# cherubicXN/neat

Measured on AMD Instinct MI355X. Metric: ray-samples/s (train step) on ABC-neat-a, higher is better.
Workload: dtype bf16; 1 GPU; C2: abc-neat-a networks, 1024 rays x 128 samples per GPU, depth samples given, train step = forward + loss + backward + Adam; rays_per_gpu=1024, samples_per_ray=128, global_rays=1024, parallelism=dp1, weights=synthetic 'rough' (seed 42), launch=hip graph replay, the whole step one launch (forward + loss + backward + Adam)

## Files before the change

### neat_amd/csrc/bf16_common.hpp

```cpp
#pragma once
#include <hip/hip_runtime.h>
#include <stdint.h>

#ifndef NEAT_HALF
#define NEAT_HALF 0
#endif

namespace neat {

struct DevOnce {
  unsigned long long mask = 0;
  static int dev() { int d = 0; if (hipGetDevice(&d) != hipSuccess || d < 0 || d > 63) d = 0; return d; }
  operator bool() const { return ((mask >> dev()) & 1ull) != 0; }
  DevOnce& operator=(bool v) { if (v) mask |= 1ull << dev(); else mask &= ~(1ull << dev()); return *this; }
};
#define NEAT_TRY(expr) do { hipError_t e_ = (expr); if (e_ != hipSuccess) return e_; } while (0)
template <auto... Kerns> hipError_t lds_limit(int bytes) {
  static DevOnce done;
  if (done) return hipSuccess;
  hipError_t e = hipSuccess;
  ((e = e != hipSuccess ? e : hipFuncSetAttribute(reinterpret_cast<const void*>(Kerns), hipFuncAttributeMaxDynamicSharedMemorySize, bytes)), ...);
  if (e == hipSuccess) done = true;
  return e;
}
// ... 80 lines not shown

struct FusedArgs {
  const float* x_fm; int P, ldp;
  const uint4* Wp[9]; int KS[9]; const float* bias[9];
  int save, values_only;
  u16* h[9];
  float* E;
  u16* feat; float* sdfraw;
  const uint4* Wlo[9]; u16* hlo[9]; u16* featlo;
  float* sdf_out;
  float radius, scale;
  int bias8_rot, bias8_n;
  const int* gate; int gate_value;
};

struct AdjArgs {
  int P, ldp;
  const uint4* Wp[8];
  const u16* h[9];
  u16* u[8];
  const float* w8; const float* rs8;
  float* es; float* e0;
  const uint4* Wlo[8]; const u16* hlo[9];
};

struct HeadX3Args {
  int P, ldp;
  int nvalid;
  const u16* feat; const u16* featlo;
  const float* small; int srows;
  const uint4* Wp[5]; const uint4* Wlo[5];
  const float* bias[5];
  u16* hid[5];
  float* out;
  const u16* smallbf;
  u16* mask[5];
};

// ... 15 lines not shown
```

### neat_amd/csrc/kernels.hpp

```cpp
#pragma once
#include <hip/hip_runtime.h>
#include <stdint.h>
#include "bf16_common.hpp"
#include "device_util.hpp"

namespace neat {

constexpr int BM = 64;
constexpr int WG = 256;

__device__ __forceinline__ float softplus100(float a) {
  const float t = 100.0f * a;
  return t > 20.0f ? a : log1pf(expf(t)) * 0.01f;
}
__device__ __forceinline__ float dphi_from_h(float h) { return -expm1f(-100.0f * h); }

enum Epi : int {
  EPI_LINEAR = 0,
  EPI_SOFTPLUS = 1,
  EPI_RELU = 2,
  EPI_SIGMOID = 3,
  EPI_REV = 4,
  EPI_TAN = 5,
  EPI_BWD = 6,
// ... 596 lines not shown
      f *= 2.0f;
    }
  }
}

__global__ void adjoint_seed_kernel(const float* __restrict__ v8, const float* __restrict__ rs8,
                                    const float* __restrict__ h8, int ldp, float* __restrict__ u7) {
  const int p = blockIdx.x * blockDim.x + threadIdx.x;
  const int n = blockIdx.y;
  if (p >= ldp) return;
  const float w = v8[n] * rs8[0];
  const size_t idx = (size_t)n * ldp + p;
  u7[idx] = w * dphi_from_h(h8[idx]);
}

struct HeadInArgs { const float* dirs; int P, S; float* small_r; float* small_a; u16* bf_r; u16* bf_a;
                    int skip_fp32 = 0; };
template <bool FAST>
__global__ void sdf_finalize_kernel(const float* __restrict__ x_fm, const float* __restrict__ out8,
                                    const float* __restrict__ e0, const float* __restrict__ es, int P, int ldp,
                                    float radius, float scale, float* __restrict__ sdf, float* __restrict__ g_fm,
                                    float* __restrict__ mask, float* __restrict__ sdf_rm, float* __restrict__ g_rm,
                                    int n_clamp, float* __restrict__ g_extra_rm, const float* __restrict__ E, HeadInArgs hin) {
  const int p = blockIdx.x * blockDim.x + threadIdx.x;
  if (p >= ldp) return;
  float xv[3], gv[3] = {0.f, 0.f, 0.f};
#pragma unroll
  for (int c = 0; c < 3; ++c) xv[c] = x_fm[(size_t)c * ldp + p];
  float s = out8[p], m = 0.0f;
  if (e0) {
#pragma unroll
    for (int c = 0; c < 3; ++c) {
      float acc = e0[(size_t)c * ldp + p] + es[(size_t)c * ldp + p];
      float f = 1.0f;
#pragma unroll
      for (int k = 0; k < 6; ++k) {
        const float es_ = e0[(size_t)(3 + 6 * k + c) * ldp + p] + es[(size_t)(3 + 6 * k + c) * ldp + p];
        const float ec_ = e0[(size_t)(6 + 6 * k + c) * ldp + p] + es[(size_t)(6 + 6 * k + c) * ldp + p];
        const float ang = xv[c] * f;
        if (E) acc += f * E[(size_t)(6 + 6 * k + c) * ldp + p] * es_ - f * E[(size_t)(3 + 6 * k + c) * ldp + p] * ec_;
        else acc += f * (FAST ? __cosf(ang) : cosf(ang)) * es_ - f * (FAST ? __sinf(ang) : sinf(ang)) * ec_;
        f *= 2.0f;
      }
      gv[c] = acc;
    }
  }
  if (radius > 0.0f && p < n_clamp) {
    const float nr = sqrtf(xv[0] * xv[0] + xv[1] * xv[1] + xv[2] * xv[2]);
    const float sph = scale * (radius - nr);
    if (sph < s) {
      s = sph; m = 1.0f;
      const float inv = nr > 0.0f ? -scale / nr : 0.0f;
      gv[0] = xv[0] * inv; gv[1] = xv[1] * inv; gv[2] = xv[2] * inv;
    }
  }
  sdf[p] = s;
  if (mask) mask[p] = m;
  if (g_fm) { g_fm[p] = gv[0]; g_fm[(size_t)ldp + p] = gv[1]; g_fm[(size_t)2 * ldp + p] = gv[2]; }
  if (hin.small_r) {
    const int r = (p < hin.P ? p : 0) / hin.S;
    float vr[40], va[16];
#pragma unroll
    for (int i = 0; i < 40; ++i) vr[i] = 0.0f;
#pragma unroll
    for (int i = 0; i < 16; ++i) va[i] = 0.0f;
#pragma unroll
    for (int c = 0; c < 3; ++c) {
      const float xc = xv[c], gc = gv[c];
      const float dc = (p < hin.P) ? hin.dirs[r * 3 + c] : 0.0f;
      vr[c] = xc; vr[3 + c] = dc;
      float f = 1.0f;
#pragma unroll
      for (int k = 0; k < 4; ++k) {
        vr[6 + 6 * k + c] = sinf(dc * f);
        vr[9 + 6 * k + c] = cosf(dc * f);
        f *= 2.0f;
      }
      vr[30 + c] = gc;
      va[c] = xc; va[3 + c] = dc; va[6 + c] = gc;
    }
    if (!hin.skip_fp32) {
#pragma unroll
      for (int i = 0; i < 33; ++i) hin.small_r[(size_t)i * ldp + p] = vr[i];
#pragma unroll
      for (int i = 0; i < 9; ++i) hin.small_a[(size_t)i * ldp + p] = va[i];
    }
    if (hin.bf_r) {
#pragma unroll
      for (int o = 0; o < 5; ++o)
        reinterpret_cast<uint4*>(hin.bf_r)[(size_t)o * ldp + p] = make_uint4(pack2(vr[8 * o], vr[8 * o + 1]), pack2(vr[8 * o + 2], vr[8 * o + 3]),
                                                                            pack2(vr[8 * o + 4], vr[8 * o + 5]), pack2(vr[8 * o + 6], vr[8 * o + 7]));
    }
    if (hin.bf_a) {
#pragma unroll
// ... 319 lines not shown
```

### neat_amd/csrc/kernels_fused.hpp

```cpp
#pragma once
#include "bf16_common.hpp"
#include "fused_launch.hpp"
#include <type_traits>

namespace neat {

#ifndef NEAT_F6_ABLATE
#define NEAT_F6_ABLATE 0
#endif
#ifndef NEAT_ADJ_ABLATE
#define NEAT_ADJ_ABLATE 0
#endif
#ifndef NEAT_ADJ_NT_LOAD
#define NEAT_ADJ_NT_LOAD 1
#endif
#ifndef NEAT_F6_WIDE
#define NEAT_F6_WIDE 1
#endif
#ifndef NEAT_ADJ_WIDE
#define NEAT_ADJ_WIDE 1
#endif
#ifndef NEAT_F6_SPLITK
#define NEAT_F6_SPLITK 0
#endif
// ... 45 lines not shown
}
__device__ __forceinline__ void f6_store16(void* p, uint4 v) {
  typedef unsigned v4u_t __attribute__((ext_vector_type(4)));
  const v4u_t w = {v.x, v.y, v.z, v.w};
  if (NEAT_F6_NT) __builtin_nontemporal_store(w, reinterpret_cast<v4u_t*>(p));
  else *reinterpret_cast<v4u_t*>(p) = w;
}
__device__ __forceinline__ void f6_store8(void* p, uint2 v) {
  typedef unsigned long long u64_t;
  if (NEAT_F6_NT) __builtin_nontemporal_store(__builtin_bit_cast(u64_t, v), reinterpret_cast<u64_t*>(p));
  else *reinterpret_cast<uint2*>(p) = v;
}

template <bool ACT_, bool SAVE_, int N_, int DST_, int BIASOFF_, bool UDOM_ = false> struct F6EpiCfg {
  static constexpr bool ACT = ACT_, SAVE = SAVE_, NONE = false, REV = false, UDOM = UDOM_;
  static constexpr int N = N_, DST = DST_, BIASOFF = BIASOFF_, SPLIT = 1 << 30;
};
struct F6NoEpi { static constexpr bool ACT = false, SAVE = false, NONE = true, REV = false, UDOM = false; static constexpr int N = 256, DST = 0, BIASOFF = 0, SPLIT = 1 << 30; };
template <bool SAVE_, int N_, int DST_, int SPLIT_> struct F6RevCfg {
  static constexpr bool ACT = false, SAVE = SAVE_, NONE = false, REV = true, UDOM = false;
  static constexpr int N = N_, DST = DST_, BIASOFF = 0, SPLIT = SPLIT_;
};

template <class E, int RT> __device__ __forceinline__ void f6_load_bias(const F6Lane& L, float4 (&bq)[4 * RT]) {
#pragma unroll
  for (int g = 0; g < 4 * RT; ++g) bq[g] = *reinterpret_cast<const float4*>(L.bias + (E::BIASOFF + (g >> 2) * 32 + 8 * (g & 3)) * 4);
}

template <class E, int RT> __device__ __forceinline__ void f6_load_bias16(const F6Lane& L, f32x16 (&c0)[RT]) {
#pragma unroll
  for (int g = 0; g < 4 * RT; ++g) {
    const float4 b = *reinterpret_cast<const float4*>(L.bias + (E::BIASOFF + (g >> 2) * 32 + 8 * (g & 3)) * 4);
    c0[g >> 2][4 * (g & 3) + 0] = b.x; c0[g >> 2][4 * (g & 3) + 1] = b.y; c0[g >> 2][4 * (g & 3) + 2] = b.z; c0[g >> 2][4 * (g & 3) + 3] = b.w;
  }
}

// ... 20 lines not shown
          }
          hw = st.hs[2 * (q & 1) + pr];
        } else hw = __float_as_uint(pr ? bq[g].y : bq[g].x);
        st.m0 = x0 * dphi_fast(bf_lo(hw));
        st.m1 = x1 * dphi_fast(bf_hi(hw));
      }
      return;
    }
    float r0 = st.m0, r1 = st.m1;
    if (E::SPLIT < 256 && 32 * (RT * wave + i) + 8 * q + 7 >= E::SPLIT) {
      int hio = hi;
      asm volatile("" : "+v"(hio));
      const int n0 = 32 * (RT * wave + i) + 8 * q + 4 * hio + 2 * pr;
      const bool st_ok = FULL || t < nt;
      const unsigned col = L.fcol + t * 32, ld = L.ldp16 >> 4;
      if (n0 >= E::SPLIT) { r0 = 0.0f; if (st_ok && n0 < E::N) f6_storef(L.frows + (unsigned)(n0 - E::SPLIT) * ld + col, x0); }
      if (n0 + 1 >= E::SPLIT) { r1 = 0.0f; if (st_ok && n0 + 1 < E::N) f6_storef(L.frows + (unsigned)(n0 + 1 - E::SPLIT) * ld + col, x1); }
    }
    const unsigned pk = pack2(r0, r1);
    if (pr == 0) { st.lo = pk; return; }
    const uint2 v = make_uint2(st.lo, pk);
    if (E::SPLIT > 0) *reinterpret_cast<uint2*>(L.quad[E::DST] + ((i * 4 + q) * BP + t * 32) * 16) = v;
    if (E::SAVE && (FULL || t < nt) && !(NEAT_ADJ_ABLATE & 1)) {
      if (NEAT_ADJ_WIDE) {
        if (q & 1) f6_store16(reinterpret_cast<char*>(hout) + ((unsigned)(i * 4 + q - 1) * L.ldp16 + L.goct) + t * 512, f6_octet(st.vprev, v));
        else st.vprev = v;
      } else f6_store8(reinterpret_cast<char*>(hout) + ((unsigned)(i * 4 + q) * L.ldp16 + L.gquad) + t * 512, v);
    }
    return;
  }
  if (h == 0) {
    if (E::ACT && NEAT_F6_ABLATE != 1) {
// ... 374 lines not shown
          sv = fminf(sv, a.scale * (a.radius - sqrtf(x0 * x0 + x1 * x1 + x2 * x2)));
        }
        if (p < a.P) a.sdf_out[p] = sv;
      } else {
        a.sdfraw[p] = sv;
      }
    }
    __syncthreads();
   }
  }
}

#ifndef NEAT_ADJ_SINGLE
#define NEAT_ADJ_SINGLE 1
#endif
template <bool SAVE>
__global__ __launch_bounds__(512, 2) void sdf_adjoint_w64_kernel(AdjArgs a, int ntiles, int nwg) {
  constexpr int NT = 4, RT = 1;
  typedef F6Cfg<NT, RT> C;
  constexpr int BP = C::BP, F6T = C::THREADS;
  extern __shared__ __attribute__((aligned(16))) unsigned char f6lds[];
  float* seedw = reinterpret_cast<float*>(f6lds + C::BIAS);
  if (NEAT_F6_PRIO == 1 && threadIdx.x >= 256) __builtin_amdgcn_s_setprio(1);
  if (NEAT_F6_PRIO == 2 && threadIdx.x < 256) __builtin_amdgcn_s_setprio(1);
  const int tid = threadIdx.x, lane = tid & 63, hi = lane >> 5;
  const int wave = __builtin_amdgcn_readfirstlane(tid >> 6);
  for (int k = tid; k < 256; k += F6T) seedw[k] = a.w8[k] * a.rs8[0];

  uint4 wA[RT][16];
  auto w_addr = [&](const uint4* Wl, int N) -> const unsigned char* {
    const int tile = (RT * wave) * 32 < N ? RT * wave : 0;
    unsigned voff = (unsigned)((tile * 16) * 64 + lane) * 16u;
    asm volatile("" : "+v"(voff));
    return reinterpret_cast<const unsigned char*>(Wl) + voff;
  };
  {
    const unsigned char* w7 = w_addr(a.Wp[7], 256);
#pragma unroll
    for (int ks = 0; ks < 16; ++ks) wA[0][ks] = *reinterpret_cast<const uint4*>(w7 + ks * 1024);
  }

  F6Lane L;
  {
    const unsigned fo = (unsigned)(hi * BP + (lane & 31)) * 16u, qo = (unsigned)((4 * RT * wave) * BP + (lane & 31)) * 16u + 8u * hi;
    unsigned b0 = fo, b1 = fo + C::XB, q0 = qo, q1 = qo + C::XB, bb = C::BIAS + (unsigned)(32 * RT * wave + 4 * hi) * 4u;
    asm volatile("" : "+v"(b0), "+v"(b1), "+v"(q0), "+v"(q1), "+v"(bb));
    L.frag[0] = f6lds + b0; L.frag[1] = f6lds + b1; L.frag[2] = f6lds + b0;
    L.quad[0] = f6lds + q0; L.quad[1] = f6lds + q1; L.bias = f6lds + bb; L.pe0 = f6lds;
  }
  L.ldp16 = (unsigned)a.ldp * 16u;
  __syncthreads();

  const int t_begin = (int)(((long long)blockIdx.x * ntiles) / nwg), t_end = (int)(((long long)(blockIdx.x + 1) * ntiles) / nwg);
  for (int tile0 = t_begin; tile0 < t_end; tile0 += NT) {
   const int ntb = min(NT, t_end - tile0);
   for (int sub = 0; sub < ((ntb == NT || !NEAT_ADJ_SINGLE) ? 1 : ntb); ++sub) {
    const int p0 = (tile0 + sub) * 32;
    const int nt = (ntb == NT || !NEAT_ADJ_SINGLE) ? ntb : 1;
    L.gquad = ((unsigned)(4 * RT * wave) * (unsigned)a.ldp + (unsigned)(p0 + (lane & 31))) * 16u + 8u * hi;
    L.goct = ((unsigned)(4 * RT * wave + hi) * (unsigned)a.ldp + (unsigned)(p0 + (lane & 31))) * 16u;
// ... 44 lines not shown
#pragma unroll
          for (int q = 0; q < 4; ++q) {
            const unsigned h0 = __float_as_uint(hq[0][q].x), h1 = __float_as_uint(hq[0][q].y);
            const uint2 v = make_uint2(pack2(wq[q].x * dphi_fast(bf_lo(h0)), wq[q].y * dphi_fast(bf_hi(h0))),
                                       pack2(wq[q].z * dphi_fast(bf_lo(h1)), wq[q].w * dphi_fast(bf_hi(h1))));
            *reinterpret_cast<uint2*>(L.quad[0] + (q * BP + t * 32) * 16) = v;
            if (SAVE) *reinterpret_cast<uint2*>(reinterpret_cast<char*>(a.u[7]) + ((unsigned)q * L.ldp16 + L.gquad) + t * 512) = v;
          }
        }
      }
      __syncthreads();

      typedef F6RevCfg<SAVE, 256, 1, 1 << 30> R7;
      typedef F6RevCfg<SAVE, 256, 0, 1 << 30> R6;
      typedef F6RevCfg<SAVE, 256, 1, 1 << 30> R5;
      typedef F6RevCfg<SAVE, 256, 0, 217> R4;
      typedef F6RevCfg<SAVE, 256, 1, 1 << 30> R3;
      typedef F6RevCfg<SAVE, 256, 0, 1 << 30> R2;
      typedef F6RevCfg<SAVE, 256, 1, 1 << 30> R1;
      typedef F6RevCfg<false, 39, 0, 0> R0;
      f32x16 acc[2][RT];
      uint4 ring[NEAT_F6_RING];
      constexpr int RD = NEAT_F6_RING;
#define ADJ_STAGE(S_, T_, SRC_, WC_, E_, H_, TE_, NFR_)                                                                              \
      f6_stage<NT, RT, FULL, true, 16, SRC_, E_, (16 * (S_)) % RD, ((S_) % 2 == 1)>(L, WC_, T_, acc[(S_) & 1], acc[((S_) + 1) & 1], hq[((S_) + HD - 1) % HD], TE_, nt, H_, wave, hi, ring, NFR_);
#define ADJ_STAGE_ROLL(S_, T_, SRC_, WC_, E_, H_, TE_, NFR_, WNX_)                                                                   \
      f6_stage<NT, RT, FULL, true, 16, SRC_, E_, (16 * (S_)) % RD, ((S_) % 2 == 1), true>(L, WC_, T_, acc[(S_) & 1], acc[((S_) + 1) & 1], hq[((S_) + HD - 1) % HD], TE_, nt, H_, wave, hi, ring, NFR_, WNX_);
#define ADJ_LAYER(S0_, SRC_, WC_, EPREV_, ECUR_, HPREV_, HCUR_, HAS_H_, HSRC_, NSRC_, FPREV_, FCUR_, WNEXT_, NNEXT_, HASN_, HNEXT_)             \
      { L.frows = FPREV_;                                                                                                         \
        if (HD == 2 && HAS_H_) load_h(hq[((S0_) + 0) % HD], HSRC_, 0);                                                              \
        if (HD == 3 && HAS_H_) load_h(hq[((S0_) + 1) % HD], HSRC_, 1);                                                              \
        ADJ_STAGE((S0_) + 0, 0, SRC_, WC_, EPREV_, HPREV_, NT - 1, L.frag[SRC_] + 1 * 512)                                         \
        if (HD == 4 && HAS_H_) load_h(hq[((S0_) + 2) % HD], HSRC_, 2);                                                              \
        L.frows = FCUR_;                                                                                                          \
        if (HD == 2 && HAS_H_) load_h(hq[((S0_) + 1) % HD], HSRC_, 1);                                                              \
// ... 49 lines not shown
        for (int q = 0; q < 4; ++q) wq[q] = *reinterpret_cast<const float4*>(L.bias + (8 * q) * 4);
        load_h(hq, a.h[8], false);
#pragma unroll
        for (int q = 0; q < 4; ++q) {
          const unsigned h0 = __float_as_uint(hq[q].x), h1 = __float_as_uint(hq[q].y);
          const uint2 v = make_uint2(pack2(wq[q].x * dphi_fast(bf_lo(h0)), wq[q].y * dphi_fast(bf_hi(h0))),
                                     pack2(wq[q].z * dphi_fast(bf_lo(h1)), wq[q].w * dphi_fast(bf_hi(h1))));
          *reinterpret_cast<uint2*>(L.quad[0] + (q * BP) * 16) = v;
          if (SAVE) *reinterpret_cast<uint2*>(reinterpret_cast<char*>(a.u[7]) + ((unsigned)q * L.ldp16 + L.gquad)) = v;
        }
      }
      __syncthreads();
      typedef F6RevCfg<SAVE, 256, 1, 1 << 30> R7;
      typedef F6RevCfg<SAVE, 256, 0, 1 << 30> R6;
      typedef F6RevCfg<SAVE, 256, 1, 1 << 30> R5;
      typedef F6RevCfg<SAVE, 256, 0, 217> R4;
      typedef F6RevCfg<SAVE, 256, 1, 1 << 30> R3;
      typedef F6RevCfg<SAVE, 256, 0, 1 << 30> R2;
      typedef F6RevCfg<SAVE, 256, 1, 1 << 30> R1;
      typedef F6RevCfg<false, 39, 0, 0> R0;
      f32x16 acc[2][RT];
      uint4 ring[NEAT_F6_RING];
      constexpr int RD = NEAT_F6_RING;
#define ADJ_LAYER1(SRC_, ECUR_, HCUR_, HAS_H_, HSRC_, FCUR_, WNEXT_, NNEXT_)                                                          \
      { _Pragma("unroll") for (int j = 0; j < RD - 1; ++j) ring[j] = *reinterpret_cast<const uint4*>(L.frag[SRC_] + j * 2 * BP * 16);  \
        if (HAS_H_) load_h(hq, HSRC_);                                                                                              \
        L.frows = FCUR_;                                                                                                            \
        f6_stage<NT, RT, FULL, true, 16, SRC_, F6NoEpi, 0, false, true>(L, wA, 0, acc[0], acc[1], hq, 0, 1, nullptr, wave, hi, ring, nullptr, w_addr(WNEXT_, NNEXT_)); \
        f6_stage<NT, RT, FULL, false, 16, 0, ECUR_, 0, true>(L, wA, 0, acc[1], acc[0], hq, 0, 1, HCUR_, wave, hi, ring, nullptr); }
      ADJ_LAYER1(0, R7, a.u[6], 1, a.h[7], nullptr, a.Wp[6], 256)
      ADJ_LAYER1(1, R6, a.u[5], 1, a.h[6], nullptr, a.Wp[5], 256)
      ADJ_LAYER1(0, R5, a.u[4], 1, a.h[5], nullptr, a.Wp[4], 256)
      ADJ_LAYER1(1, R4, a.u[3], 1, a.h[4], a.es, a.Wp[3], 256)
      ADJ_LAYER1(0, R3, a.u[2], 1, a.h[3], nullptr, a.Wp[2], 256)
      ADJ_LAYER1(1, R2, a.u[1], 1, a.h[2], nullptr, a.Wp[1], 256)
      ADJ_LAYER1(0, R1, a.u[0], 1, a.h[1], nullptr, a.Wp[0], 39)
      ADJ_LAYER1(1, R0, nullptr, 0, a.h[1], a.e0, a.Wp[7], 256)
#undef ADJ_LAYER1
    };
#ifndef NEAT_ADJ_ONE_VARIANT
#define NEAT_ADJ_ONE_VARIANT 1
#endif
    if (NEAT_ADJ_SINGLE && ntb != NT) chain_single();
    else if (NEAT_ADJ_ONE_VARIANT) chain(std::false_type{});
    else if (nt == NT) chain(std::true_type{});
    else chain(std::false_type{});
    __syncthreads();
   }
  }
}

}
```

### neat_amd/csrc/neat_fused.hip

```cpp
#if defined(NEAT_HALF) && NEAT_HALF
#define neat neat_f16
#endif
#include "kernels_fused.hpp"
#include "kernels_x3.hpp"
#include "kernels_heads.hpp"

namespace neat {

hipError_t launch_sdf_fused_w64(hipStream_t st, const FusedArgs& a, int ntiles, int nwg, bool full) {
  typedef F6Cfg<4, 1> C;
  NEAT_TRY((lds_limit<&sdf_fused_w64_kernel<4, false, 1>, &sdf_fused_w64_kernel<4, true, 1>>(C::LDS)));
  if (full) hipLaunchKernelGGL((sdf_fused_w64_kernel<4, false, 1>), dim3(nwg), dim3(C::THREADS), C::LDS, st, a, ntiles, nwg);
  else hipLaunchKernelGGL((sdf_fused_w64_kernel<4, true, 1>), dim3(nwg), dim3(C::THREADS), C::LDS, st, a, ntiles, nwg);
  return hipGetLastError();
}

hipError_t launch_sdf_adjoint_w64(hipStream_t st, const AdjArgs& a, int ntiles, int nwg, bool save) {
  typedef F6Cfg<4, 1> C;
  NEAT_TRY((lds_limit<&sdf_adjoint_w64_kernel<true>, &sdf_adjoint_w64_kernel<false>>(C::LDS)));
  if (save) hipLaunchKernelGGL((sdf_adjoint_w64_kernel<true>), dim3(nwg), dim3(C::THREADS), C::LDS, st, a, ntiles, nwg);
  else hipLaunchKernelGGL((sdf_adjoint_w64_kernel<false>), dim3(nwg), dim3(C::THREADS), C::LDS, st, a, ntiles, nwg);
  return hipGetLastError();
}

template <auto Kern, class A> static hipError_t x3_launch(hipStream_t st, int nbatches, int nwg, const A& args) {
  NEAT_TRY(lds_limit<Kern>(X3::LDS));
  const int grid = nbatches < nwg ? nbatches : nwg;
  if (grid <= 0) return hipSuccess;
  hipLaunchKernelGGL(Kern, dim3(grid), dim3(X3::THREADS), X3::LDS, st, args, nbatches);
  return hipGetLastError();
}

hipError_t launch_sdf_chain_x3(hipStream_t st, const FusedArgs& a, int nbatches, int nwg, bool full) {
// ... 32 lines not shown
```

### neat_amd/csrc/neat_net.hip

```cpp
#include <mutex>
#include <unordered_map>
#if defined(NEAT_HALF) && NEAT_HALF
#define neat neat_f16
#include "f16_symbols.h"
#endif
#include "kernels_bf16.hpp"
#include "kernels_dw.hpp"
#include "fused_launch.hpp"
#include "../../include/neat_hip.h"
#include <algorithm>
#include <initializer_list>
#include <utility>
#include <math.h>
#include <stdio.h>
#include <stdlib.h>
#include <vector>

using namespace neat;

namespace {

constexpr int L_REND = 9, L_ATTR = 14;
const int kO[NLAYERS] = {256, 256, 256, 217, 256, 256, 256, 256, 257, 256, 256, 256, 256, 3, 256, 256, 256, 256, 6};
const int kI[NLAYERS] = {39, 256, 256, 256, 256, 256, 256, 256, 256, 289, 256, 256, 256, 256, 265, 256, 256, 256, 256};
// ... 133 lines not shown
  hipLaunchKernelGGL((layer_kernel_h<EPI, PT, OBF>), dim3(a.ldp / BMT), dim3(WG), lds, st, a);
  return hipGetLastError();
}
template <int EPI> hipError_t launch_layer_h(hipStream_t st, const LayerArgsH& a, int) {
  if (a.out0_bf16) return g_pt_bf16 == 4 ? launch_layer_h_pt<EPI, 4, true>(st, a) : launch_layer_h_pt<EPI, 2, true>(st, a);
  return launch_layer_h_pt<EPI, 2, false>(st, a);
}
int g_wgrad_batch = -1;
inline int wgrad_batch_size(int ldp) {
  if (g_wgrad_batch >= 0) return g_wgrad_batch;
  return ldp <= 200000 ? 3 : (ldp <= 400000 ? 2 : 0);
}
int g_wreduce_direct = 2;
int g_head_chain = 2;
int g_fused_adj = 1;
int g_layer_ws = 1;
constexpr int WS_GRID = 256;
constexpr int DW_MAXGRID = 256;
inline int dw_slots(int ldp) {
  const int nt = ldp / WSP;
  return nt < DW_MAXGRID ? (nt > 0 ? nt : 1) : DW_MAXGRID;
}
inline int dw_grid(int ldp) {
  const int nt = ldp / WSP;
  return nt < DW_MAXGRID ? nt : DW_MAXGRID;
}
int g_ws_aux_nt = 15;
int g_ws_wide_store = 1;
const int* g_gate = nullptr; int g_gate_value = 0;
int g_ws_interleave = 1;
// ... 359 lines not shown
    hipError_t e6 = launch_sdf_fused_w64(c.st, a, ntiles, ntiles < WS_GRID ? ntiles : WS_GRID, full);
    prof_end(c.st, ps);
    return e6;
  }
  hipLaunchKernelGGL(posenc6_kernel, grid1(c.ldp), dim3(256), 0, c.st, w.x, c.ldp, w.E);
  hipError_t e;
  for (int l = 0; l < 8; ++l) {
    In a = l == 0 ? in(F(w.E), PE_ROWS) : in(w.h[l], l == 4 ? 217 : 256);
    In b = l == 4 ? in(F(w.E), PE_ROWS) : NOIN;
    if ((e = layer(c, L.fwd[l], EPI_SOFTPLUS, a, b, c.net->b[l], kO[l], w.h[l + 1])) != hipSuccess) return e;
  }
  if (!full) return layer(c, L.sdf_row, EPI_LINEAR, in(w.h[8], 256), NOIN, c.net->b[8], 1, F(w.sdfraw));
  return layer(c, L.fwd[8], EPI_LINEAR, in(w.h[8], 256), NOIN, c.net->b[8], 257, F(w.sdfraw));
}

hipError_t sdf_adjoint(const Ctx& c, const SdfWs& w, bool save = true) {
  const PackLayout& L = c.L();
  if (c.prec && (g_fused_adj || c.hx3)) {
    AdjArgs a{};
    a.P = c.P; a.ldp = c.ldp;
    for (int l = 0; l < 8; ++l) {
      const PackDesc2& d = L.d[L.tr[l]];
      if (d.Kpad != 256) return hipErrorInvalidValue;
      a.Wp[l] = reinterpret_cast<const uint4*>(c.packed + d.offset);
      a.u[l] = reinterpret_cast<u16*>(w.u[l].p);
    }
    for (int l = 1; l <= 8; ++l) a.h[l] = reinterpret_cast<const u16*>(w.h[l].p);
    a.w8 = c.net->v[8]; a.rs8 = c.rowscale(8); a.es = w.es; a.e0 = w.e0;
    const int ntiles = c.ldp / 32;
    const int nwg = ntiles < WS_GRID ? ntiles : WS_GRID;
    double fl = 0.0;
    for (int l = 0; l < 8; ++l) fl += 2.0 * kO[l] * kI[l] * (double)c.P;
    if (c.hx3) {
      for (int l = 0; l < 8; ++l) a.Wlo[l] = reinterpret_cast<const uint4*>(c.packed + L.d[L.tr_lo[l]].offset);
      for (int l = 1; l <= 8; ++l) a.hlo[l] = reinterpret_cast<const u16*>(w.hlo[l].p);
      ProfSlot* ps3 = prof_begin(c.st, 3, fl, (double)c.P * (2 * 8 * 512.0 + (save ? 8 * 512.0 : 0.0) + 2 * 39 * 4.0) + 4.0 * 589000.0);
      hipError_t e3 = launch_sdf_adjoint_x3(c.st, a, c.ldp / X3_BATCH, WS_GRID, save);
      prof_end(c.st, ps3);
      return e3;
    }
    ProfSlot* ps = prof_begin(c.st, 3, fl, (double)c.P * (8 * 512.0 + (save ? 8 * 512.0 : 0.0) + 2 * 39 * 4.0) + 2.0 * 589000.0);
    hipError_t e = launch_sdf_adjoint_w64(c.st, a, ntiles, nwg, save);
    prof_end(c.st, ps);
    return e;
  }
  if (c.prec)
    hipLaunchKernelGGL(adjoint_seed_kernel_h, dim3((c.ldp + 255) / 256, 32), dim3(256), 0, c.st, c.net->v[8], c.rowscale(8),
                       reinterpret_cast<const u16*>(w.h[8].p), c.ldp, reinterpret_cast<u16*>(w.u[7].p));
  else
    hipLaunchKernelGGL(adjoint_seed_kernel, dim3((c.ldp + 255) / 256, 256), dim3(256), 0, c.st, c.net->v[8], c.rowscale(8),
                       w.h[8].f(), c.ldp, w.u[7].f());
  hipError_t e;
  for (int l = 7; l >= 1; --l) {
    if (l == 4) {
      e = layer(c, L.tr[l], EPI_REV, in(w.u[l], kO[l]), NOIN, nullptr, 256, w.u[l - 1], F(w.es), 217, w.h[l]);
    } else {
// ... 795 lines not shown
  if (key == 1 && (value == 0 || value == 1)) { g_wgrad_h3 = value; return 0; }
  if (key == 2 && (value == 0 || value == 1)) { g_layer_ws = value; return 0; }
  if (key == 6 && value >= 0 && value <= 2) { g_wreduce_direct = value; return 0; }
  if (key == 8 && (value == -1 || value == 0 || value == 2 || value == 3 || value == 6)) { g_wgrad_batch = value; return 0; }
  if (key == 9 && value >= 0 && value <= 2) { g_ws_interleave = value; return 0; }
  if (key == 11 && value >= 0 && value <= 63) { g_ws_aux_nt = value; return 0; }
  if (key == 12 && (value == 0 || value == 1)) { g_ws_wide_store = value; return 0; }
  if (key == 13 && (value == 0 || value == 1)) { g_fused_adj = value; return 0; }
  if (key == 14 && value >= 0 && value <= 2) { g_head_chain = value; return 0; }
  if (key == 16 && value >= 0 && value <= 2) { g_dw_fused = value; return 0; }
  if (key == 17 && value >= 0 && value <= 7) { g_dw_ablate = value; return 0; }
  if (key == 21 && value >= 0 && value <= 4) { g_wgrad_narrow = value; return 0; }
  if (key == 22 && (value == 0 || value == 1)) { g_dw_lin8 = value; return 0; }
  if (key == 24 && (value == 0 || value == 1)) { g_chain_pp = value; return 0; }
  if (key == 25 && (value == 0 || value == 1)) { g_dw_segments = value; return 0; }
  return -1;
}

int neat_prof_enable(int on) {
#if !NEAT_HALF
  f16_neat_prof_enable(on);
#endif
  g_prof.on = on != 0;
  g_prof.used = 0;
  return 0;
}

int neat_prof_collect(int cls, double* total_ms, double* total_flops, int* launches, double* total_bytes) {
  double ms = 0.0, fl = 0.0, by = 0.0;
  int n = 0;
// ... 75 lines not shown
  else if (x) hipLaunchKernelGGL(rm_to_fm_kernel, grid1(c.ldp), dim3(256), 0, c.st, x, P, 3, c.ldp, w.x);
  else hipLaunchKernelGGL(points_from_rays_kernel, grid1(c.ldp), dim3(256), 0, c.st, rp->origins, rp->dirs, rp->z, rp->R, rp->S, c.ldp, w.x,
                          (float*)nullptr, (const float*)nullptr, 0);
  if (mode == 0 && pr.prec) {
    NEAT_CHECK(sdf_primal(c, w, false, radius, scale, sdf));
    return (int)hipGetLastError();
  }
  if (mode == 0) {
    NEAT_CHECK(sdf_primal(c, w, false));
    FINALIZE_LAUNCH(c, w.x, w.sdfraw, (const float*)nullptr,
                       (const float*)nullptr, P, c.ldp, radius, scale, w.sdf, (float*)nullptr, (float*)nullptr, sdf, (float*)nullptr,
                       P, (float*)nullptr);
    return (int)hipGetLastError();
  }
  NEAT_CHECK(sdf_primal(c, w, true));
  NEAT_CHECK(sdf_adjoint(c, w));
  FINALIZE_LAUNCH(c, w.x, w.sdfraw, w.e0, w.es, P, c.ldp, radius, scale,
                     w.sdf, w.g, w.mask, sdf, grad, P, (float*)nullptr);
  export_out8(c, w, out257, feat);
  return (int)hipGetLastError();
}

int neat_sdf_forward(const float* packed, const neat_net_params* net, const float* x, int P, int mode, int precision,
                     float radius, float scale, float* ws, float* out257, float* sdf, float* feat, float* grad,
                     void* stream) {
  NEAT_F16_FWD(neat_sdf_forward(packed, net, x, P, mode, precision, radius, scale, ws, out257, sdf, feat, grad, stream))
  if (P > 0 && !x) return -1;
  return sdf_forward_impl(packed, net, x, nullptr, P, mode, precision, radius, scale, ws, out257, sdf, feat, grad, stream);
}

int neat_sdf_values_rays(const float* packed, const neat_net_params* net, const float* origins, const float* dirs, const float* z, int R,
                         int S, int precision, float radius, float scale, float* ws, float* sdf, const int* gate, int gate_value,
                         void* stream) {
// ... 115 lines not shown
static int render_forward_impl(const float* packed, const neat_net_params* net, const float* origins, const float* dirs,
                               const float* z, int R, int S, int precision, const float* beta, float beta_min, float radius, float scale, float* ws,
                               float* points, float* weights, float* sdf, float* rgb, float* lines3d, float* depth,
                               float* xyz, float* normal_map, const float* eik_points, int E, float* eik_grad, void* stream, bool fwd_only) {
  const Prec pr = resolve(precision);
  if (pr.hx3 == 2) return -1;
  if (R <= 0 || S <= 0) return 0;
  if (!packed || !net || !ws || !origins || !dirs || !z || !rgb || !lines3d || !depth || !xyz || !pr.ok) return -1;
  if (E < 0 || (E > 0 && (!eik_points || !eik_grad))) return -1;
  const int Pm = R * S, P = Pm + E;
  Ctx c = make_ctx(pr, packed, net, P, stream);
  SdfWs w = sdf_ws(ws, c.ldp, fwd_only ? 2 : 1, pr.prec, pr.hx3);
  HeadWs h = head_ws(ws + w.total, c.ldp, pr.prec, fwd_only);
  hipLaunchKernelGGL(points_from_rays_kernel, grid1(c.ldp), dim3(256), 0, c.st, origins, dirs, z, R, S, c.ldp, w.x, points, eik_points, E);
  NEAT_CHECK(sdf_primal(c, w, true));
  NEAT_CHECK(sdf_adjoint(c, w, !fwd_only));
  HeadInArgs hin{dirs, Pm, S, h.small_r, h.small_a, reinterpret_cast<u16*>(h.smallbf_r.p), reinterpret_cast<u16*>(h.smallbf_a.p)};
  hin.skip_fp32 = (oct_operands(c) && !c.hx3) ? 1 : 0;
  FINALIZE_LAUNCH_H(c, hin, w.x, w.sdfraw, w.e0, w.es, P, c.ldp, radius, scale,
                    w.sdf, w.g, w.mask, sdf, (float*)nullptr, Pm, eik_grad);
  NEAT_CHECK(heads_forward(c, h, w.feat, w.featlo, !fwd_only, Pm));
  CompositeArgs ca;
  ca.z = z; ca.sdf = w.sdf; ca.dirs = dirs; ca.x_fm = w.x; ca.rgb_fm = h.rgb; ca.lin_fm = h.lin; ca.g_fm = w.g;
  ca.R = R; ca.S = S; ca.ldp = c.ldp; ca.beta_ptr = beta; ca.beta_min = beta_min;
  ca.weights = weights; ca.rgb = rgb; ca.lines3d = lines3d; ca.depth = depth; ca.xyz = xyz; ca.normal_map = normal_map;
  hipLaunchKernelGGL(composite_fwd_kernel, dim3((R + 3) / 4), dim3(WG), 0, c.st, ca);
  return (int)hipGetLastError();
}

int neat_render_forward(const float* packed, const neat_net_params* net, const float* origins, const float* dirs,
                        const float* z, int R, int S, int precision, const float* beta, float beta_min, float radius, float scale, float* ws,
                        float* points, float* weights, float* sdf, float* rgb, float* lines3d, float* depth,
                        float* xyz, float* normal_map, const float* eik_points, int E, float* eik_grad, void* stream) {
  NEAT_F16_FWD(neat_render_forward(packed, net, origins, dirs, z, R, S, precision, beta, beta_min, radius, scale, ws, points, weights, sdf, rgb, lines3d, depth, xyz, normal_map, eik_points, E, eik_grad, stream))
  return render_forward_impl(packed, net, origins, dirs, z, R, S, precision, beta, beta_min, radius, scale, ws, points, weights, sdf, rgb, lines3d,
// ... 60 lines not shown
```

Before: 50.24 million ray-samples/s.

## Fold SDF finalize into the fused adjoint kernel epilogue via LDS stashes

```diff
diff --git a/neat_amd/csrc/bf16_common.hpp b/neat_amd/csrc/bf16_common.hpp
--- a/neat_amd/csrc/bf16_common.hpp
+++ b/neat_amd/csrc/bf16_common.hpp
@@ -118,6 +118,16 @@
   const int* gate; int gate_value;
 };
 
+struct HeadInArgs { const float* dirs; int P, S; float* small_r; float* small_a; u16* bf_r; u16* bf_a;
+                    int skip_fp32 = 0; };
+
+struct FinArgs {
+  int on;
+  const float* x_fm; const float* out8; int P, n_clamp; float radius, scale;
+  float* sdf; float* g_fm; float* mask; float* sdf_rm; float* g_rm; float* g_extra_rm;
+  HeadInArgs hin;
+};
+
 struct AdjArgs {
   int P, ldp;
   const uint4* Wp[8];
@@ -126,6 +136,7 @@
   const float* w8; const float* rs8;
   float* es; float* e0;
   const uint4* Wlo[8]; const u16* hlo[9];
+  FinArgs fin;
 };
 
 struct HeadX3Args {
diff --git a/neat_amd/csrc/kernels.hpp b/neat_amd/csrc/kernels.hpp
--- a/neat_amd/csrc/kernels.hpp
+++ b/neat_amd/csrc/kernels.hpp
@@ -3,6 +3,7 @@
 #include <stdint.h>
 #include "bf16_common.hpp"
 #include "device_util.hpp"
+#include "sdf_finalize.hpp"
 
 namespace neat {
 
@@ -634,8 +635,6 @@
   u7[idx] = w * dphi_from_h(h8[idx]);
 }
 
-struct HeadInArgs { const float* dirs; int P, S; float* small_r; float* small_a; u16* bf_r; u16* bf_a;
-                    int skip_fp32 = 0; };
 template <bool FAST>
 __global__ void sdf_finalize_kernel(const float* __restrict__ x_fm, const float* __restrict__ out8,
                                     const float* __restrict__ e0, const float* __restrict__ es, int P, int ldp,
@@ -650,29 +649,12 @@
   float s = out8[p], m = 0.0f;
   if (e0) {
 #pragma unroll
-    for (int c = 0; c < 3; ++c) {
-      float acc = e0[(size_t)c * ldp + p] + es[(size_t)c * ldp + p];
-      float f = 1.0f;
-#pragma unroll
-      for (int k = 0; k < 6; ++k) {
-        const float es_ = e0[(size_t)(3 + 6 * k + c) * ldp + p] + es[(size_t)(3 + 6 * k + c) * ldp + p];
-        const float ec_ = e0[(size_t)(6 + 6 * k + c) * ldp + p] + es[(size_t)(6 + 6 * k + c) * ldp + p];
-        const float ang = xv[c] * f;
-        if (E) acc += f * E[(size_t)(6 + 6 * k + c) * ldp + p] * es_ - f * E[(size_t)(3 + 6 * k + c) * ldp + p] * ec_;
-        else acc += f * (FAST ? __cosf(ang) : cosf(ang)) * es_ - f * (FAST ? __sinf(ang) : sinf(ang)) * ec_;
-        f *= 2.0f;
-      }
-      gv[c] = acc;
-    }
-  }
-  if (radius > 0.0f && p < n_clamp) {
-    const float nr = sqrtf(xv[0] * xv[0] + xv[1] * xv[1] + xv[2] * xv[2]);
-    const float sph = scale * (radius - nr);
-    if (sph < s) {
-      s = sph; m = 1.0f;
-      const float inv = nr > 0.0f ? -scale / nr : 0.0f;
-      gv[0] = xv[0] * inv; gv[1] = xv[1] * inv; gv[2] = xv[2] * inv;
-    }
+    for (int c = 0; c < 3; ++c)
+      gv[c] = fin_normal_comp<FAST>(c, xv[c], [&](int j) { return e0[(size_t)j * ldp + p] + es[(size_t)j * ldp + p]; }, E, ldp, p);
+  }
+  float inv;
+  if (fin_sphere_clamp(xv[0], xv[1], xv[2], radius, scale, p < n_clamp, s, m, inv)) {
+    gv[0] = xv[0] * inv; gv[1] = xv[1] * inv; gv[2] = xv[2] * inv;
   }
   sdf[p] = s;
   if (mask) mask[p] = m;
@@ -686,18 +668,9 @@
     for (int i = 0; i < 16; ++i) va[i] = 0.0f;
 #pragma unroll
     for (int c = 0; c < 3; ++c) {
-      const float xc = xv[c], gc = gv[c];
       const float dc = (p < hin.P) ? hin.dirs[r * 3 + c] : 0.0f;
-      vr[c] = xc; vr[3 + c] = dc;
-      float f = 1.0f;
-#pragma unroll
-      for (int k = 0; k < 4; ++k) {
-        vr[6 + 6 * k + c] = sinf(dc * f);
-        vr[9 + 6 * k + c] = cosf(dc * f);
-        f *= 2.0f;
-      }
-      vr[30 + c] = gc;
-      va[c] = xc; va[3 + c] = dc; va[6 + c] = gc;
+      fin_head_comp(c, xv[c], dc, gv[c], [&](int i, float v) { vr[i] = v; });
+      va[c] = xv[c]; va[3 + c] = dc; va[6 + c] = gv[c];
     }
     if (!hin.skip_fp32) {
 #pragma unroll
diff --git a/neat_amd/csrc/kernels_fused.hpp b/neat_amd/csrc/kernels_fused.hpp
--- a/neat_amd/csrc/kernels_fused.hpp
+++ b/neat_amd/csrc/kernels_fused.hpp
@@ -1,6 +1,7 @@
 #pragma once
 #include "bf16_common.hpp"
 #include "fused_launch.hpp"
+#include "sdf_finalize.hpp"
 #include <type_traits>
 
 namespace neat {
@@ -83,12 +84,13 @@
 
 template <bool ACT_, bool SAVE_, int N_, int DST_, int BIASOFF_, bool UDOM_ = false> struct F6EpiCfg {
   static constexpr bool ACT = ACT_, SAVE = SAVE_, NONE = false, REV = false, UDOM = UDOM_;
-  static constexpr int N = N_, DST = DST_, BIASOFF = BIASOFF_, SPLIT = 1 << 30;
+  static constexpr int N = N_, DST = DST_, BIASOFF = BIASOFF_, SPLIT = 1 << 30, FST = -1;
+  static constexpr bool FGLOB = true;
 };
-struct F6NoEpi { static constexpr bool ACT = false, SAVE = false, NONE = true, REV = false, UDOM = false; static constexpr int N = 256, DST = 0, BIASOFF = 0, SPLIT = 1 << 30; };
-template <bool SAVE_, int N_, int DST_, int SPLIT_> struct F6RevCfg {
-  static constexpr bool ACT = false, SAVE = SAVE_, NONE = false, REV = true, UDOM = false;
-  static constexpr int N = N_, DST = DST_, BIASOFF = 0, SPLIT = SPLIT_;
+struct F6NoEpi { static constexpr bool ACT = false, SAVE = false, NONE = true, REV = false, UDOM = false; static constexpr int N = 256, DST = 0, BIASOFF = 0, SPLIT = 1 << 30, FST = -1; static constexpr bool FGLOB = true; };
+template <bool SAVE_, int N_, int DST_, int SPLIT_, int FST_ = -1, bool FGLOB_ = true> struct F6RevCfg {
+  static constexpr bool ACT = false, SAVE = SAVE_, NONE = false, REV = true, UDOM = false, FGLOB = FGLOB_;
+  static constexpr int N = N_, DST = DST_, BIASOFF = 0, SPLIT = SPLIT_, FST = FST_;
 };
 
 template <class E, int RT> __device__ __forceinline__ void f6_load_bias(const F6Lane& L, float4 (&bq)[4 * RT]) {
@@ -139,8 +141,14 @@
       const int n0 = 32 * (RT * wave + i) + 8 * q + 4 * hio + 2 * pr;
       const bool st_ok = FULL || t < nt;
       const unsigned col = L.fcol + t * 32, ld = L.ldp16 >> 4;
-      if (n0 >= E::SPLIT) { r0 = 0.0f; if (st_ok && n0 < E::N) f6_storef(L.frows + (unsigned)(n0 - E::SPLIT) * ld + col, x0); }
-      if (n0 + 1 >= E::SPLIT) { r1 = 0.0f; if (st_ok && n0 + 1 < E::N) f6_storef(L.frows + (unsigned)(n0 + 1 - E::SPLIT) * ld + col, x1); }
+      if (n0 >= E::SPLIT) { r0 = 0.0f; if (E::FGLOB && st_ok && n0 < E::N) f6_storef(L.frows + (unsigned)(n0 - E::SPLIT) * ld + col, x0); }
+      if (n0 + 1 >= E::SPLIT) { r1 = 0.0f; if (E::FGLOB && st_ok && n0 + 1 < E::N) f6_storef(L.frows + (unsigned)(n0 + 1 - E::SPLIT) * ld + col, x1); }
+      if (E::FST >= 0) {
+        extern __shared__ __attribute__((aligned(16))) unsigned char f6lds[];
+        float* fs = reinterpret_cast<float*>(f6lds + E::FST) + ((L.fcol & 31u) + t * 32);
+        if (st_ok && n0 >= E::SPLIT && n0 < E::N) fs[(n0 - E::SPLIT) * BP] = x0;
+        if (st_ok && n0 + 1 >= E::SPLIT && n0 + 1 < E::N) fs[(n0 + 1 - E::SPLIT) * BP] = x1;
+      }
     }
     const unsigned pk = pack2(r0, r1);
     if (pr == 0) { st.lo = pk; return; }
@@ -545,13 +553,17 @@
 #ifndef NEAT_ADJ_SINGLE
 #define NEAT_ADJ_SINGLE 1
 #endif
-template <bool SAVE>
+template <bool SAVE, bool FIN = false>
 __global__ __launch_bounds__(512, 2) void sdf_adjoint_w64_kernel(AdjArgs a, int ntiles, int nwg) {
   constexpr int NT = 4, RT = 1;
   typedef F6Cfg<NT, RT> C;
   constexpr int BP = C::BP, F6T = C::THREADS;
+  constexpr int FIN_ROWS = 39 * BP * 4;
+  constexpr int FIN_E0 = C::XA, FIN_ES = C::PE, FIN_VR = C::XB;
+  constexpr int SEED = FIN ? C::PE + FIN_ROWS : C::BIAS;
+  static_assert(SEED + 256 * 4 <= C::LDS && FIN_ROWS <= C::XBYTES, "the stashes fit the chain's LDS layout");
   extern __shared__ __attribute__((aligned(16))) unsigned char f6lds[];
-  float* seedw = reinterpret_cast<float*>(f6lds + C::BIAS);
+  float* seedw = reinterpret_cast<float*>(f6lds + SEED);
   if (NEAT_F6_PRIO == 1 && threadIdx.x >= 256) __builtin_amdgcn_s_setprio(1);
   if (NEAT_F6_PRIO == 2 && threadIdx.x < 256) __builtin_amdgcn_s_setprio(1);
   const int tid = threadIdx.x, lane = tid & 63, hi = lane >> 5;
@@ -574,7 +586,7 @@
   F6Lane L;
   {
     const unsigned fo = (unsigned)(hi * BP + (lane & 31)) * 16u, qo = (unsigned)((4 * RT * wave) * BP + (lane & 31)) * 16u + 8u * hi;
-    unsigned b0 = fo, b1 = fo + C::XB, q0 = qo, q1 = qo + C::XB, bb = C::BIAS + (unsigned)(32 * RT * wave + 4 * hi) * 4u;
+    unsigned b0 = fo, b1 = fo + C::XB, q0 = qo, q1 = qo + C::XB, bb = SEED + (unsigned)(32 * RT * wave + 4 * hi) * 4u;
     asm volatile("" : "+v"(b0), "+v"(b1), "+v"(q0), "+v"(q1), "+v"(bb));
     L.frag[0] = f6lds + b0; L.frag[1] = f6lds + b1; L.frag[2] = f6lds + b0;
     L.quad[0] = f6lds + q0; L.quad[1] = f6lds + q1; L.bias = f6lds + bb; L.pe0 = f6lds;
@@ -649,11 +661,11 @@
       typedef F6RevCfg<SAVE, 256, 1, 1 << 30> R7;
       typedef F6RevCfg<SAVE, 256, 0, 1 << 30> R6;
       typedef F6RevCfg<SAVE, 256, 1, 1 << 30> R5;
-      typedef F6RevCfg<SAVE, 256, 0, 217> R4;
+      typedef F6RevCfg<SAVE, 256, 0, 217, FIN ? FIN_ES : -1, SAVE || !FIN> R4;
       typedef F6RevCfg<SAVE, 256, 1, 1 << 30> R3;
       typedef F6RevCfg<SAVE, 256, 0, 1 << 30> R2;
       typedef F6RevCfg<SAVE, 256, 1, 1 << 30> R1;
-      typedef F6RevCfg<false, 39, 0, 0> R0;
+      typedef F6RevCfg<false, 39, 0, 0, FIN ? FIN_E0 : -1, SAVE || !FIN> R0;
       f32x16 acc[2][RT];
       uint4 ring[NEAT_F6_RING];
       constexpr int RD = NEAT_F6_RING;
@@ -733,11 +745,11 @@
       typedef F6RevCfg<SAVE, 256, 1, 1 << 30> R7;
       typedef F6RevCfg<SAVE, 256, 0, 1 << 30> R6;
       typedef F6RevCfg<SAVE, 256, 1, 1 << 30> R5;
-      typedef F6RevCfg<SAVE, 256, 0, 217> R4;
+      typedef F6RevCfg<SAVE, 256, 0, 217, FIN ? FIN_ES : -1, SAVE || !FIN> R4;
       typedef F6RevCfg<SAVE, 256, 1, 1 << 30> R3;
       typedef F6RevCfg<SAVE, 256, 0, 1 << 30> R2;
       typedef F6RevCfg<SAVE, 256, 1, 1 << 30> R1;
-      typedef F6RevCfg<false, 39, 0, 0> R0;
+      typedef F6RevCfg<false, 39, 0, 0, FIN ? FIN_E0 : -1, SAVE || !FIN> R0;
       f32x16 acc[2][RT];
       uint4 ring[NEAT_F6_RING];
       constexpr int RD = NEAT_F6_RING;
@@ -764,6 +776,65 @@
     else if (NEAT_ADJ_ONE_VARIANT) chain(std::false_type{});
     else if (nt == NT) chain(std::true_type{});
     else chain(std::false_type{});
+    if constexpr (FIN) {
+      typedef const __attribute__((address_space(4))) unsigned char* kptr_t;
+      kptr_t kp = (kptr_t)__builtin_amdgcn_kernarg_segment_ptr();
+      asm volatile("" : "+s"(kp));
+      const FinArgs F = *(const FinArgs*)(kp + offsetof(AdjArgs, fin));
+      const int np = nt * 32, ldp = a.ldp;
+      const bool heads = F.hin.small_r != nullptr;
+      float* vrs = reinterpret_cast<float*>(f6lds + FIN_VR);
+      if (tid < 3 * BP && (tid & (BP - 1)) < np) {
+        const int c = tid / BP, pp = tid & (BP - 1), p = p0 + pp;
+        const float* e0s = reinterpret_cast<const float*>(f6lds + FIN_E0) + pp;
+        const float* ess = reinterpret_cast<const float*>(f6lds + FIN_ES) + pp;
+        const float x0 = F.x_fm[p], x1 = F.x_fm[(size_t)ldp + p], x2 = F.x_fm[(size_t)2 * ldp + p];
+        const float xc = c == 0 ? x0 : (c == 1 ? x1 : x2);
+        float s = F.out8[p], m = 0.0f, inv;
+        float g = fin_normal_comp<true>(c, xc, [&](int j) { return e0s[j * BP] + ess[j * BP]; }, nullptr, ldp, p);
+        if (fin_sphere_clamp(x0, x1, x2, F.radius, F.scale, p < F.n_clamp, s, m, inv)) g = xc * inv;
+        if (c == 0) {
+          F.sdf[p] = s;
+          if (F.mask) F.mask[p] = m;
+        }
+        if (F.g_fm) F.g_fm[(size_t)c * ldp + p] = g;
+        if (heads) {
+          const HeadInArgs& H = F.hin;
+          const int r = (p < H.P ? p : 0) / H.S;
+          const float dc = (p < H.P) ? H.dirs[r * 3 + c] : 0.0f;
+          fin_head_comp(c, xc, dc, g, [&](int i, float v) {
+            vrs[i * BP + pp] = v;
+            if (!H.skip_fp32) H.small_r[(size_t)i * ldp + p] = v;
+          });
+          if (!H.skip_fp32) { H.small_a[(size_t)c * ldp + p] = xc; H.small_a[(size_t)(3 + c) * ldp + p] = dc; H.small_a[(size_t)(6 + c) * ldp + p] = g; }
+        }
+        if (p < F.P) {
+          if (p < F.n_clamp) {
+            if (c == 0 && F.sdf_rm) F.sdf_rm[p] = s;
+            if (F.g_rm) F.g_rm[p * 3 + c] = g;
+          } else if (F.g_extra_rm) {
+            F.g_extra_rm[(p - F.n_clamp) * 3 + c] = g;
+          }
+        }
+      }
+      __syncthreads();
+      if (heads) {
+        const HeadInArgs& H = F.hin;
+        for (int j = tid; j < 7 * BP; j += F6T) {
+          const int pp = j & (BP - 1), o = j / BP;
+          if (pp >= np) continue;
+          float v[8];
+#pragma unroll
+          for (int i = 0; i < 8; ++i) {
+            const int row = o < 5 ? 8 * o + i : (o == 5 ? (i < 6 ? i : 24 + i) : (i == 0 ? 32 : 33));
+            v[i] = row < 33 ? vrs[row * BP + pp] : 0.0f;
+          }
+          const size_t p = (size_t)(p0 + pp);
+          if (o < 5) { if (H.bf_r) reinterpret_cast<uint4*>(H.bf_r)[(size_t)o * ldp + p] = fin_pack8(v); }
+          else if (H.bf_a) reinterpret_cast<uint4*>(H.bf_a)[(size_t)(o - 5) * ldp + p] = fin_pack8(v);
+        }
+      }
+    }
     __syncthreads();
    }
   }
diff --git a/neat_amd/csrc/neat_fused.hip b/neat_amd/csrc/neat_fused.hip
--- a/neat_amd/csrc/neat_fused.hip
+++ b/neat_amd/csrc/neat_fused.hip
@@ -17,6 +17,12 @@
 
 hipError_t launch_sdf_adjoint_w64(hipStream_t st, const AdjArgs& a, int ntiles, int nwg, bool save) {
   typedef F6Cfg<4, 1> C;
+  if (a.fin.on) {
+    NEAT_TRY((lds_limit<&sdf_adjoint_w64_kernel<true, true>, &sdf_adjoint_w64_kernel<false, true>>(C::LDS)));
+    if (save) hipLaunchKernelGGL((sdf_adjoint_w64_kernel<true, true>), dim3(nwg), dim3(C::THREADS), C::LDS, st, a, ntiles, nwg);
+    else hipLaunchKernelGGL((sdf_adjoint_w64_kernel<false, true>), dim3(nwg), dim3(C::THREADS), C::LDS, st, a, ntiles, nwg);
+    return hipGetLastError();
+  }
   NEAT_TRY((lds_limit<&sdf_adjoint_w64_kernel<true>, &sdf_adjoint_w64_kernel<false>>(C::LDS)));
   if (save) hipLaunchKernelGGL((sdf_adjoint_w64_kernel<true>), dim3(nwg), dim3(C::THREADS), C::LDS, st, a, ntiles, nwg);
   else hipLaunchKernelGGL((sdf_adjoint_w64_kernel<false>), dim3(nwg), dim3(C::THREADS), C::LDS, st, a, ntiles, nwg);
diff --git a/neat_amd/csrc/neat_net.hip b/neat_amd/csrc/neat_net.hip
--- a/neat_amd/csrc/neat_net.hip
+++ b/neat_amd/csrc/neat_net.hip
@@ -171,6 +171,7 @@
 int g_wreduce_direct = 2;
 int g_head_chain = 2;
 int g_fused_adj = 1;
+int g_fin_fold = 1;
 int g_layer_ws = 1;
 constexpr int WS_GRID = 256;
 constexpr int DW_MAXGRID = 256;
@@ -560,7 +561,8 @@
   return layer(c, L.fwd[8], EPI_LINEAR, in(w.h[8], 256), NOIN, c.net->b[8], 257, F(w.sdfraw));
 }
 
-hipError_t sdf_adjoint(const Ctx& c, const SdfWs& w, bool save = true) {
+hipError_t sdf_adjoint(const Ctx& c, const SdfWs& w, bool save = true, const FinArgs* fin = nullptr, bool* folded = nullptr) {
+  if (folded) *folded = false;
   const PackLayout& L = c.L();
   if (c.prec && (g_fused_adj || c.hx3)) {
     AdjArgs a{};
@@ -585,7 +587,11 @@
       prof_end(c.st, ps3);
       return e3;
     }
-    ProfSlot* ps = prof_begin(c.st, 3, fl, (double)c.P * (8 * 512.0 + (save ? 8 * 512.0 : 0.0) + 2 * 39 * 4.0) + 2.0 * 589000.0);
+    const bool fold = fin && g_fin_fold;
+    if (fold) { a.fin = *fin; a.fin.on = 1; }
+    if (folded) *folded = fold;
+    const double fin_bytes = !fold ? 2 * 39 * 4.0 : (save ? 2 * 39 * 4.0 : 0.0) + 4 * 4.0 + 5 * 4.0 + (fin->hin.small_r ? 7 * 16.0 : 0.0);
+    ProfSlot* ps = prof_begin(c.st, 3, fl, (double)c.P * (8 * 512.0 + (save ? 8 * 512.0 : 0.0) + fin_bytes) + 2.0 * 589000.0);
     hipError_t e = launch_sdf_adjoint_w64(c.st, a, ntiles, nwg, save);
     prof_end(c.st, ps);
     return e;
@@ -1411,6 +1417,7 @@
   if (key == 22 && (value == 0 || value == 1)) { g_dw_lin8 = value; return 0; }
   if (key == 24 && (value == 0 || value == 1)) { g_chain_pp = value; return 0; }
   if (key == 25 && (value == 0 || value == 1)) { g_dw_segments = value; return 0; }
+  if (key == 31 && (value == 0 || value == 1)) { g_fin_fold = value; return 0; }
   return -1;
 }
 
@@ -1516,9 +1523,12 @@
     return (int)hipGetLastError();
   }
   NEAT_CHECK(sdf_primal(c, w, true));
-  NEAT_CHECK(sdf_adjoint(c, w));
-  FINALIZE_LAUNCH(c, w.x, w.sdfraw, w.e0, w.es, P, c.ldp, radius, scale,
-                     w.sdf, w.g, w.mask, sdf, grad, P, (float*)nullptr);
+  FinArgs fin{0, w.x, w.sdfraw, P, P, radius, scale, w.sdf, w.g, w.mask, sdf, grad, nullptr, HeadInArgs{}};
+  bool folded;
+  NEAT_CHECK(sdf_adjoint(c, w, true, &fin, &folded));
+  if (!folded)
+    FINALIZE_LAUNCH(c, w.x, w.sdfraw, w.e0, w.es, P, c.ldp, radius, scale,
+                       w.sdf, w.g, w.mask, sdf, grad, P, (float*)nullptr);
   export_out8(c, w, out257, feat);
   return (int)hipGetLastError();
 }
@@ -1664,11 +1674,14 @@
   HeadWs h = head_ws(ws + w.total, c.ldp, pr.prec, fwd_only);
   hipLaunchKernelGGL(points_from_rays_kernel, grid1(c.ldp), dim3(256), 0, c.st, origins, dirs, z, R, S, c.ldp, w.x, points, eik_points, E);
   NEAT_CHECK(sdf_primal(c, w, true));
-  NEAT_CHECK(sdf_adjoint(c, w, !fwd_only));
   HeadInArgs hin{dirs, Pm, S, h.small_r, h.small_a, reinterpret_cast<u16*>(h.smallbf_r.p), reinterpret_cast<u16*>(h.smallbf_a.p)};
   hin.skip_fp32 = (oct_operands(c) && !c.hx3) ? 1 : 0;
-  FINALIZE_LAUNCH_H(c, hin, w.x, w.sdfraw, w.e0, w.es, P, c.ldp, radius, scale,
-                    w.sdf, w.g, w.mask, sdf, (float*)nullptr, Pm, eik_grad);
+  FinArgs fin{0, w.x, w.sdfraw, P, Pm, radius, scale, w.sdf, w.g, w.mask, sdf, nullptr, eik_grad, hin};
+  bool folded;
+  NEAT_CHECK(sdf_adjoint(c, w, !fwd_only, &fin, &folded));
+  if (!folded)
+    FINALIZE_LAUNCH_H(c, hin, w.x, w.sdfraw, w.e0, w.es, P, c.ldp, radius, scale,
+                      w.sdf, w.g, w.mask, sdf, (float*)nullptr, Pm, eik_grad);
   NEAT_CHECK(heads_forward(c, h, w.feat, w.featlo, !fwd_only, Pm));
   CompositeArgs ca;
   ca.z = z; ca.sdf = w.sdf; ca.dirs = dirs; ca.x_fm = w.x; ca.rgb_fm = h.rgb; ca.lin_fm = h.lin; ca.g_fm = w.g;
diff --git a/neat_amd/csrc/sdf_finalize.hpp b/neat_amd/csrc/sdf_finalize.hpp
--- /dev/null
+++ b/neat_amd/csrc/sdf_finalize.hpp
@@ -0,0 +1,53 @@
+#pragma once
+#include "bf16_common.hpp"
+
+namespace neat {
+
+template <bool FAST, class EE>
+__device__ __forceinline__ float fin_normal_comp(int c, float xc, EE ee, const float* __restrict__ E, int ldp, int p) {
+  float acc = ee(c);
+  float f = 1.0f;
+#pragma unroll
+  for (int k = 0; k < 6; ++k) {
+    const float es_ = ee(3 + 6 * k + c);
+    const float ec_ = ee(6 + 6 * k + c);
+    const float ang = xc * f;
+    if (E) acc += f * E[(size_t)(6 + 6 * k + c) * ldp + p] * es_ - f * E[(size_t)(3 + 6 * k + c) * ldp + p] * ec_;
+    else acc += f * (FAST ? __cosf(ang) : cosf(ang)) * es_ - f * (FAST ? __sinf(ang) : sinf(ang)) * ec_;
+    f *= 2.0f;
+  }
+  return acc;
+}
+
+__device__ __forceinline__ bool fin_sphere_clamp(float x0, float x1, float x2, float radius, float scale, bool clamp_point, float& s,
+                                                 float& m, float& inv) {
+  if (radius > 0.0f && clamp_point) {
+    const float nr = sqrtf(x0 * x0 + x1 * x1 + x2 * x2);
+    const float sph = scale * (radius - nr);
+    if (sph < s) {
+      s = sph; m = 1.0f;
+      inv = nr > 0.0f ? -scale / nr : 0.0f;
+      return true;
+    }
+  }
+  return false;
+}
+
+template <class Put>
+__device__ __forceinline__ void fin_head_comp(int c, float xc, float dc, float gc, Put put) {
+  put(c, xc); put(3 + c, dc);
+  float f = 1.0f;
+#pragma unroll
+  for (int k = 0; k < 4; ++k) {
+    put(6 + 6 * k + c, sinf(dc * f));
+    put(9 + 6 * k + c, cosf(dc * f));
+    f *= 2.0f;
+  }
+  put(30 + c, gc);
+}
+
+__device__ __forceinline__ uint4 fin_pack8(const float (&v)[8]) {
+  return make_uint4(pack2(v[0], v[1]), pack2(v[2], v[3]), pack2(v[4], v[5]), pack2(v[6], v[7]));
+}
+
+}
```

New measurement: 50.04 million ray-samples/s. About the same (-0.4%).
